# kabkabm/defensegan

Hardware: NVIDIA H100
Metric: reconstructed images/sec at R=10,L=200 (higher is better)
Workload: dtype f16

## Files before the change

### defensegan_b200/csrc/kernels_tc2.cuh

```cuda
#pragma once
#include "kernels_tc.cuh"
#include "tc_records.cuh"

namespace dgan {

constexpr int TC2_SMEM_MAX = 232448;
constexpr int TC2_TILE_BYTES = 128 * 128;
constexpr int TC2_BUF_COLS = 256;
constexpr int TC2_CONSUMERS = 256;
constexpr int TC2_THREADS = TC2_CONSUMERS + 128;
constexpr int TC2_PRODUCER_REGS = 40, TC2_CONSUMER_REGS = 232;
constexpr int TC2_STORE_ROWS = 16;

constexpr int TC2_MAX_PAIRS = 80;
struct Tc2Heads {
  uint32_t off[TC2_MAX_PAIRS + 1];
};

struct __align__(16) TcItem2 {
  uint16_t q[16];
  uint32_t n_acc;
};
static_assert(sizeof(TcItem2) == 48 && offsetof(TcItem2, n_acc) == 32, "the kernel's item loads");

__host__ __device__ constexpr int tc2_acc_stride(int n_tile) { return n_tile <= 32 ? 32 : (n_tile < 64 ? 64 : n_tile); }

__host__ __device__ constexpr bool tc2_tma_epilogue(int n_tile, int epi, int out_bytes) {
  return out_bytes == 2 && n_tile >= 64 && epi != EPI_FINAL_SIGMOID1 && epi != EPI_FINAL_TANH3 && epi != EPI_FINAL_SIGMOID1_W &&
         epi != EPI_FINAL_TANH3_W;
}

constexpr int TC2_REC_BATCH = 16;
constexpr int TC2_STAGING_BYTES = TC2_REC_BATCH * (int)sizeof(TcRec);
constexpr int TC2_MREC_BYTES = TC2_NSLOT * (int)sizeof(TcRec);

__host__ __device__ constexpr int tc2_epi_tiles(int n_tile, int epi, int out_bytes) {
  return tc2_tma_epilogue(n_tile, epi, out_bytes) ? 2 : 0;
}
__host__ __device__ constexpr int tc2_ksub(int K) { return K % 64 == 0 ? 4 : K / 16; }
__host__ __device__ constexpr int tc2_a_bytes(int ksub) { return 128 * 32 * ksub; }
__host__ __device__ constexpr int tc2_b_bytes(int n_tile, int ksub) { return n_tile * 32 * ksub; }
__host__ __device__ constexpr bool tc2_issues_zero_ops(int maxb, int ksub) { return maxb > 4 || (maxb > 1 && ksub < 4); }
__host__ __device__ constexpr int tc2_zero_bytes(int n_tile, int maxb, int ksub) { return maxb > 1 ? tc2_b_bytes(n_tile, ksub) : 0; }
__host__ __device__ constexpr int tc2_ring_bytes(int n_tile, int maxb, int ksub, int epi, int out_bytes) {
  const int epi_b = tc2_epi_tiles(n_tile, epi, out_bytes) * TC2_TILE_BYTES;
  const int raw = ((TC2_SMEM_MAX - 1024 - 256 - TC2_MREC_BYTES - TC2_STAGING_BYTES - epi_b - tc2_zero_bytes(n_tile, maxb, ksub)) / 1024) * 1024;
  return raw > TC2_RING_MAX_KB * 1024 ? TC2_RING_MAX_KB * 1024 : raw;
}

template <int N_TILE, int MAXB_, int KSUB_ = 4, int EPI = EPI_NONE, int OUT_BYTES = 2>
struct Tc2Cfg {
  static_assert(MAXB_ >= 1 && MAXB_ <= TC2_BUF_COLS / tc2_acc_stride(N_TILE), "more accumulator slots than columns");
  static_assert(KSUB_ >= 1 && KSUB_ <= 4, "k16 MMAs per op");
  static constexpr int KSUB = KSUB_;
  static constexpr int A_BYTES = tc2_a_bytes(KSUB);
  static constexpr int B_TILE = tc2_b_bytes(N_TILE, KSUB);
  static constexpr int A_SUB = 128 * 32, B_SUB = N_TILE * 32;
  static constexpr int MAXB = MAXB_;
  static constexpr int ACC_REGS = MAXB * N_TILE / 2;
  static constexpr bool TMA_EPI = tc2_tma_epilogue(N_TILE, EPI, OUT_BYTES);
  static constexpr int EPI_TILES = tc2_epi_tiles(N_TILE, EPI, OUT_BYTES);
  static constexpr int EPI_BYTES = EPI_TILES * TC2_TILE_BYTES;
  static constexpr int ZERO_BYTES = tc2_zero_bytes(N_TILE, MAXB, KSUB);
  static constexpr int RING_BYTES = tc2_ring_bytes(N_TILE, MAXB, KSUB, EPI, OUT_BYTES);
  static constexpr int SMEM_BYTES = RING_BYTES + ZERO_BYTES + EPI_BYTES + TC2_STAGING_BYTES + 1024 + 256 + TC2_MREC_BYTES;
};

#define TC2_KINDS(X)                                                                                                   \
  X(256, 1, 4, EPI_BIAS_RELU, __half) X(256, 1, 4, EPI_BIAS, __half) X(256, 1, 4, EPI_MASK, __half)                    \
  X(256, 1, 4, EPI_NONE, __half) X(256, 1, 4, EPI_NONE, float) X(256, 1, 4, EPI_BIAS, float)                           \
  X(128, 2, 4, EPI_BIAS_RELU, __half) X(128, 2, 4, EPI_BIAS, __half) X(128, 2, 4, EPI_MASK, __half)                    \
  X(128, 2, 4, EPI_NONE, __half) X(128, 2, 4, EPI_NONE, float) X(128, 2, 4, EPI_BIAS, float)                           \
  X(128, 1, 4, EPI_NONE, float)                                                                                        \
  X(64, 4, 4, EPI_BIAS_RELU, __half) X(64, 4, 4, EPI_BIAS, __half) X(64, 4, 4, EPI_MASK, __half)                      \
  X(64, 4, 4, EPI_NONE, __half) X(64, 4, 4, EPI_NONE, float) X(64, 4, 4, EPI_BIAS, float)                              \
  X(64, 4, 1, EPI_MASK, __half) X(64, 4, 1, EPI_NONE, __half) X(64, 4, 3, EPI_NONE, __half)                            \
  X(128, 2, 1, EPI_MASK, __half) X(128, 2, 1, EPI_NONE, __half) X(128, 2, 3, EPI_NONE, __half)                         \
  X(16, 8, 4, EPI_FINAL_SIGMOID1, __half) X(16, 4, 4, EPI_FINAL_SIGMOID1, __half) X(48, 4, 4, EPI_FINAL_TANH3, __half)   \
  X(16, 8, 4, EPI_NONE, float) X(48, 4, 4, EPI_NONE, float)                                                              \
  X(16, 8, 4, EPI_FINAL_SIGMOID1_W, __half) X(16, 4, 4, EPI_FINAL_SIGMOID1_W, __half) X(48, 4, 4, EPI_FINAL_TANH3_W, __half)

struct Tc2Kind { int n, maxb, ksub, epi, out_bytes; };
#define TC2_KIND_ROW(NT, MB, KS, EP, T) {NT, MB, KS, EP, (int)sizeof(T)},
static constexpr Tc2Kind kTc2Kinds[] = {TC2_KINDS(TC2_KIND_ROW)};
#undef TC2_KIND_ROW
constexpr bool tc2_kinds_fit_records() {
  for (const Tc2Kind& k : kTc2Kinds)
    if ((uint32_t)k.maxb > TcMmaRec::MaxB::mask || (uint32_t)k.ksub > TcMmaRec::Ksub::mask) return false;
  return true;
}
static_assert(tc2_kinds_fit_records(), "an instantiation's MAXB or KSUB does not fit the MMA record");
static inline bool tc2_has_kind(int n, int maxb, int ksub, int epi, int out_bytes) {
  for (const Tc2Kind& k : kTc2Kinds)
    if (k.n == n && k.maxb == maxb && k.ksub == ksub && k.epi == epi && k.out_bytes == out_bytes) return true;
  return false;
}

namespace ptx {
__device__ __forceinline__ void tma_store_3d(const CUtensorMap* map, uint32_t src, int c0, int c1, int c2) {
  asm volatile("cp.async.bulk.tensor.3d.global.shared::cta.tile.bulk_group [%0, {%2, %3, %4}], [%1];"
               ::"l"(map), "r"(src), "r"(c0), "r"(c1), "r"(c2) : "memory");
}
__device__ __forceinline__ void bulk_commit() { asm volatile("cp.async.bulk.commit_group;" ::: "memory"); }
__device__ __forceinline__ void bulk_wait_read1() { asm volatile("cp.async.bulk.wait_group.read 1;" ::: "memory"); }
__device__ __forceinline__ void bulk_wait_all0() { asm volatile("cp.async.bulk.wait_group 0;" ::: "memory"); }
__device__ __forceinline__ void fence_proxy_async_smem() { asm volatile("fence.proxy.async.shared::cta;" ::: "memory"); }
__device__ __forceinline__ uint32_t cluster_ctarank() {
  uint32_t r;
  asm volatile("mov.u32 %0, %%cluster_ctarank;" : "=r"(r));
  return r;
}
__device__ __forceinline__ void cluster_sync() {
  asm volatile("barrier.cluster.arrive.release.aligned;\n\tbarrier.cluster.wait.acquire.aligned;" ::: "memory");
}
__device__ __forceinline__ void tma_load_3d_mc2(uint32_t dst, const CUtensorMap* map, uint32_t bar, int c0, int c1, int c2) {
  asm volatile(
      "cp.async.bulk.tensor.3d.shared::cluster.global.mbarrier::complete_tx::bytes.multicast::cluster [%0], [%1, {%3, %4, %5}], [%2], %6;"
      ::"r"(dst), "l"(map), "r"(bar), "r"(c0), "r"(c1), "r"(c2), "h"((uint16_t)3) : "memory");
}
__device__ __forceinline__ void mbar_arrive_cluster(uint32_t local_bar, uint32_t cta) {
  asm volatile(
      "{\n\t.reg .b32 ra;\n\t"
      "mapa.shared::cluster.u32 ra, %0, %1;\n\t"
      "mbarrier.arrive.shared::cluster.b64 _, [ra];\n\t}" ::"r"(local_bar), "r"(cta) : "memory");
}
__device__ __forceinline__ void named_bar_sync(uint32_t id, uint32_t nthreads) {
  asm volatile("bar.sync %0, %1;" ::"r"(id), "r"(nthreads) : "memory");
}
__device__ __forceinline__ void st_shared_v4(uint32_t addr, uint32_t a, uint32_t b, uint32_t c, uint32_t d) {
  asm volatile("st.shared.v4.b32 [%0], {%1, %2, %3, %4};" ::"r"(addr), "r"(a), "r"(b), "r"(c), "r"(d) : "memory");
}
__device__ __forceinline__ void st_shared_u32(uint32_t addr, uint32_t v) { asm volatile("st.shared.b32 [%0], %1;" ::"r"(addr), "r"(v) : "memory"); }
__device__ __forceinline__ uint32_t ld_shared_u32(uint32_t addr) {
  uint32_t v;
  asm volatile("ld.shared.b32 %0, [%1];" : "=r"(v) : "r"(addr) : "memory");
  return v;
}
__device__ __forceinline__ uint2 ld_shared_v2(uint32_t addr) {
  uint2 v;
  asm volatile("ld.shared.v2.b32 {%0, %1}, [%2];" : "=r"(v.x), "=r"(v.y) : "r"(addr));
  return v;
}
__device__ __forceinline__ uint4 ld_shared_v4(uint32_t addr) {
  uint4 v;
  asm volatile("ld.shared.v4.b32 {%0, %1, %2, %3}, [%4];" : "=r"(v.x), "=r"(v.y), "=r"(v.z), "=r"(v.w) : "r"(addr));
  return v;
}
__device__ __forceinline__ uint4 ld_shared_v4_ordered(uint32_t addr) {
  uint4 v;
  asm volatile("ld.shared.v4.b32 {%0, %1, %2, %3}, [%4];" : "=r"(v.x), "=r"(v.y), "=r"(v.z), "=r"(v.w) : "r"(addr) : "memory");
  return v;
}
__device__ __forceinline__ void bulk_load(uint32_t dst, const void* src, uint32_t bytes, uint32_t bar) {
  asm volatile("cp.async.bulk.shared::cluster.global.mbarrier::complete_tx::bytes [%0], [%1], %2, [%3];"
               ::"r"(dst), "l"(src), "r"(bytes), "r"(bar) : "memory");
}
__device__ __forceinline__ void wgmma_wait1() { asm volatile("wgmma.wait_group.sync.aligned 1;" ::: "memory"); }
template <int R> __device__ __forceinline__ void setmaxnreg_inc() { asm volatile("setmaxnreg.inc.sync.aligned.u32 %0;" ::"n"(R)); }
template <int R> __device__ __forceinline__ void setmaxnreg_dec() { asm volatile("setmaxnreg.dec.sync.aligned.u32 %0;" ::"n"(R)); }
__device__ __forceinline__ bool elect_one() {
  uint32_t pred;
  asm volatile("{\n\t.reg .pred P1;\n\telect.sync _|P1, 0xffffffff;\n\tselp.u32 %0, 1, 0, P1;\n\t}" : "=r"(pred));
  return pred != 0;
}
}

__device__ __forceinline__ int tc2_item_at(const int* __restrict__ order, int k, int pair, int n_pairs, int n_slots) {
  return k < n_slots ? __ldg(order + (size_t)k * n_pairs + pair) : -1;
}

template <int NT, int MAXB, int KSUB, uint32_t MASK, int NREG>
__device__ __forceinline__ void tc2_mma_ops(float (&acc)[NREG], const uint32_t (&q)[6], uint64_t da0, uint64_t db0, uint32_t zoff) {
  constexpr uint32_t DA_K = KSUB == 4 ? 2u : (uint32_t)(128 * 32 >> 4), DB_K = KSUB == 4 ? 2u : (uint32_t)(NT * 32 >> 4);
#pragma unroll
  for (int a = 0; a < MAXB; ++a) {
    if (!((MASK >> a) & 1u)) continue;
    const uint32_t e = TcMmaRec::Ops::get(q[a / TcMmaRec::Ops::PER_WORD], a);
    const uint32_t bs = TcOp::Slot::get(e);
    const uint64_t da = da0 + (uint64_t)(TcOp::A::get(e) * (uint32_t)(tc2_a_bytes(KSUB) >> 4));
    const uint32_t boff = bs * (uint32_t)(tc2_b_bytes(NT, KSUB) >> 4);
    const uint64_t db = db0 + (uint64_t)(tc2_issues_zero_ops(MAXB, KSUB) && bs == (uint32_t)TC2_ZERO_SLOT ? zoff : boff);
    const uint32_t keep = TcOp::First::get(e) ^ 1u;
#pragma unroll
    for (int k = 0; k < KSUB; ++k) ptx::Wgmma<NT>::mma(acc + a * (NT / 2), da + DA_K * k, db + DB_K * k, k > 0 ? 1u : keep);
  }
  ptx::wgmma_commit();
}

template <int NT, int MAXB, int KSUB, int NREG>
__device__ __forceinline__ void tc2_mma_round(float (&acc)[NREG], const uint32_t (&q)[6], uint64_t da0, uint64_t db0, uint32_t zoff) {
  if constexpr (tc2_issues_zero_ops(MAXB, KSUB) || MAXB == 1) {
    tc2_mma_ops<NT, MAXB, KSUB, (1u << MAXB) - 1u>(acc, q, da0, db0, zoff);
  } else {
    static_assert(MAXB <= TcMmaRec::Ops::PER_WORD, "a round's op bytes share the queue's first word");
    uint32_t set = 0;
#pragma unroll
    for (int a = 0; a < MAXB; ++a)
      set |= (TcOp::Slot::get(TcMmaRec::Ops::get(q[0], a)) != (uint32_t)TC2_ZERO_SLOT ? 1u : 0u) << a;
    switch (set) {
#define TC2_ROUND_VARIANT(M) \
  case M:                    \
    if constexpr (M < (1u << MAXB)) tc2_mma_ops<NT, MAXB, KSUB, M>(acc, q, da0, db0, zoff); \
    break;
      TC2_ROUND_VARIANT(1u) TC2_ROUND_VARIANT(2u) TC2_ROUND_VARIANT(3u) TC2_ROUND_VARIANT(4u) TC2_ROUND_VARIANT(5u)
      TC2_ROUND_VARIANT(6u) TC2_ROUND_VARIANT(7u) TC2_ROUND_VARIANT(8u) TC2_ROUND_VARIANT(9u) TC2_ROUND_VARIANT(10u)
      TC2_ROUND_VARIANT(11u) TC2_ROUND_VARIANT(12u) TC2_ROUND_VARIANT(13u) TC2_ROUND_VARIANT(14u) TC2_ROUND_VARIANT(15u)
#undef TC2_ROUND_VARIANT
      default: __builtin_unreachable();
    }
  }
}

template <int MAXB>
__device__ __forceinline__ void tc2_pop_round(uint32_t (&q)[6]) {
  using Ops = TcMmaRec::Ops;
  static_assert(Ops::WORDS == 6, "the op queue holds every op word");
  if constexpr (MAXB >= Ops::PER_WORD) {
#pragma unroll
    for (int i = 0; i < 6; ++i) q[i] = (i + MAXB / Ops::PER_WORD < 6) ? q[i + MAXB / Ops::PER_WORD] : 0u;
  } else {
#pragma unroll
    for (int i = 0; i < 5; ++i) q[i] = __funnelshift_r(q[i], q[i + 1], Ops::BITS * MAXB);
    q[5] >>= Ops::BITS * MAXB;
  }
}

#ifdef DGAN_PROBE
constexpr int TC2_PROBE_WORDS = 16;
__device__ unsigned long long g_tc2_probe[48][160][TC2_PROBE_WORDS];
__device__ __forceinline__ unsigned long long probe_gtime() {
  unsigned long long t;
  asm volatile("mov.u64 %0, %%globaltimer;" : "=l"(t));
  return t;
}
__device__ __forceinline__ long long probe_clock_after(uint32_t w0) {
  long long t;
  asm volatile("{\n\t.reg .pred p;\n\tsetp.ge.s32 p, %1, 0;\n\tmov.u64 %0, 0;\n\t@p mov.u64 %0, %%clock64;\n\t}" : "=l"(t) : "r"(w0) : "memory");
  return t;
}
__host__ __device__ constexpr int tc2_probe_key(int n_tile, int epi, int out_bytes) {
  return (n_tile == 256 ? 0 : n_tile == 128 ? 1 : n_tile == 64 ? 2 : n_tile == 48 ? 3 : 4) * 8 + (out_bytes == 4 ? 6 : (epi < 4 ? epi : epi - 4));
}
#endif

template <int N_TILE, int MAXB, int KSUB, int EPI, typename TOUT>
__global__ void __cluster_dims__(2, 1, 1) __launch_bounds__(TC2_THREADS, 1)
tc_bsgemm2_kernel(const __grid_constant__ CUtensorMap tm_a, const __grid_constant__ CUtensorMap tm_b,
                  const __grid_constant__ CUtensorMap tm_out,
                  const TcItem2* __restrict__ items, const TcRec* __restrict__ stream_p,
                  const TcRec* __restrict__ stream_m, const __grid_constant__ Tc2Heads heads,
                  const int* __restrict__ eitems, int n_slots,
                  TOUT* __restrict__ out, int n_pad, const float* __restrict__ bias, int bias_pstride, const TcFinalArgs fa) {
  using Cfg = Tc2Cfg<N_TILE, MAXB, KSUB, EPI, (int)sizeof(TOUT)>;
  constexpr bool TMA_EPI = Cfg::TMA_EPI;
  constexpr bool WEIGHTED = (EPI == EPI_FINAL_SIGMOID1_W || EPI == EPI_FINAL_TANH3_W);
  constexpr bool FINAL = (EPI == EPI_FINAL_SIGMOID1 || EPI == EPI_FINAL_TANH3 || WEIGHTED);
  constexpr bool SIGMOID1 = (EPI == EPI_FINAL_SIGMOID1 || EPI == EPI_FINAL_SIGMOID1_W);
  constexpr bool HAS_BIAS = (EPI == EPI_BIAS_RELU || EPI == EPI_BIAS);
  constexpr int B_TILE = Cfg::B_TILE, A_BYTES = Cfg::A_BYTES;
  constexpr int PRODUCER = TC2_CONSUMERS / 32;
  extern __shared__ uint8_t smem_raw[];
#ifdef DGAN_PROBE
  const long long probe_t_start = clock64();
  const unsigned long long probe_g_start = probe_gtime();
  long long probe_wait_full = 0, probe_issue = 0, probe_wait1 = 0, probe_wait0 = 0, probe_epi = 0;
  unsigned probe_rec = 0, probe_head = 0, probe_steps = 0;
#endif
  const uint32_t smem_base = (ptx::smem_u32(smem_raw) + 1023u) & ~1023u;
  const uint32_t zero_base = smem_base + Cfg::RING_BYTES;
  const uint32_t epi_base = zero_base + Cfg::ZERO_BYTES;
  const uint32_t stg_base = epi_base + Cfg::EPI_BYTES;
  const uint32_t bar_base = stg_base + TC2_STAGING_BYTES;
  const uint32_t bar_full = bar_base, bar_empty = bar_base + 64, mrec_base = bar_base + 256;

  const int warp = threadIdx.x >> 5, lane = threadIdx.x & 31;
  const uint32_t rank = ptx::cluster_ctarank();
  const int pair = blockIdx.x >> 1, n_pairs = gridDim.x >> 1;
  const uint32_t rbeg = heads.off[pair], rend = heads.off[pair + 1];

  uint4 mine = make_uint4(0, 0, 0, 0);
  if (warp == PRODUCER) {
    if (2 * rbeg + lane < 2 * rend) mine = __ldg(reinterpret_cast<const uint4*>(stream_p + rbeg) + lane);
    if (lane == 0) {
      ptx::prefetch_tmap(&tm_a);
      ptx::prefetch_tmap(&tm_b);
      if (TMA_EPI) ptx::prefetch_tmap(&tm_out);
      for (int s = 0; s < TC2_NSLOT; ++s) {
        ptx::mbar_init(bar_full + 8 * s, 1);
        ptx::mbar_init(bar_empty + 8 * s, 2 * TC2_CONSUMERS / 32);
      }
      ptx::fence_barrier_init();
    }
  }
  if constexpr (Cfg::ZERO_BYTES > 0 && tc2_issues_zero_ops(MAXB, KSUB)) {
    if (threadIdx.x < TC2_CONSUMERS) {
      for (uint32_t i = threadIdx.x; i < (uint32_t)Cfg::ZERO_BYTES / 16u; i += TC2_CONSUMERS) ptx::st_shared_v4(zero_base + 16u * i, 0u, 0u, 0u, 0u);
      ptx::fence_proxy_async_smem();
    }
  }
  ptx::cluster_sync();
#ifdef DGAN_PROBE
  const long long probe_t_entry = clock64();
#endif
  pdl_launch_dependents();
  pdl_wait();
#ifdef DGAN_PROBE
  const long long probe_t_go = clock64();
  unsigned probe_h0 = (unsigned)probe_t_go;
  bool probe_new_item = true;
#endif

  if (warp >= PRODUCER) {
    ptx::setmaxnreg_dec<TC2_PRODUCER_REGS>();
    if (warp == PRODUCER) {
      const TcRec* __restrict__ stream = stream_p;
      uint32_t it = 0;
      const uint32_t ring = stg_base;
      for (uint32_t base = rbeg; base < rend; base += TC2_REC_BATCH) {
        ptx::st_shared_v4(ring + lane * 16u, mine.x, mine.y, mine.z, mine.w);
        __syncwarp();
        if (2 * (base + TC2_REC_BATCH) + lane < 2 * rend) mine = __ldg(reinterpret_cast<const uint4*>(stream + base + TC2_REC_BATCH) + lane);
        const uint32_t cnt = min((uint32_t)TC2_REC_BATCH, rend - base);
        for (uint32_t i = 0; i < cnt; ++i, ++it) {
          const uint4 r0 = ptx::ld_shared_v4(ring + i * 32u);
          const uint2 r1 = ptx::ld_shared_v2(ring + i * 32u + 16u);
          const uint32_t slot = it & (TC2_NSLOT - 1);
          using P = TcProducerRec;
          const int kc = P::Kc::get(r0.x), nA = P::NA::get(r0.x), nB = P::NB::get(r0.x);
          const uint32_t dep = (r0.x >> P::Dep::shift) & P::Dep::mask;
          const int row0 = (2 * (int)P::Mp::get(r0.y) + (int)rank) * kRowTile;
          if (it >= dep) ptx::mbar_wait(bar_empty + 8 * ((it - dep) & (TC2_NSLOT - 1)), ((it - dep) >> 3) & 1);
          if (dep != TC2_NSLOT && it >= TC2_NSLOT) ptx::mbar_wait(bar_empty + 8 * slot, ((it - TC2_NSLOT) >> 3) & 1);
          const uint32_t full = bar_full + 8 * slot;
          const uint32_t sa = smem_base + (P::Off::get(r0.x) << 10);
          if (ptx::elect_one()) {
            ptx::mbar_expect_tx(full, (uint32_t)(nA * A_BYTES + nB * B_TILE) + (uint32_t)sizeof(TcRec));
            ptx::bulk_load(mrec_base + slot * (uint32_t)sizeof(TcRec), stream_m + rbeg + it, (uint32_t)sizeof(TcRec), full);
#pragma unroll
            for (int a = 0; a < TC2_MAX_A; ++a) {
              if (a >= nA) break;
              const int p = (int)P::Pix::get(a < P::Pix::PER_WORD ? r0.z : r0.w, a);
              if constexpr (KSUB == 4) {
                ptx::tma_load_3d(sa + a * A_BYTES, &tm_a, full, kc * 64, row0, p);
              } else {
#pragma unroll
                for (int k = 0; k < KSUB; ++k)
                  ptx::tma_load_3d(sa + a * A_BYTES + k * Cfg::A_SUB, &tm_a, full, (kc * KSUB + k) * 16, row0, p);
              }
            }
            const uint32_t sb = sa + nA * A_BYTES;
#pragma unroll
            for (int b = 0; b < TC2_MAX_BSLOTS; ++b) {
              if (b >= nB) break;
              const uint32_t t = P::Tile::get(b < P::Tile::PER_WORD ? r1.x : r1.y, b);
              if constexpr (KSUB == 4) {
                ptx::tma_load_3d_mc2(sb + b * B_TILE + rank * (B_TILE / 2), &tm_b, full, kc * 64, (int)rank * (N_TILE / 2), (int)t);
              } else {
#pragma unroll
                for (int k = 0; k < KSUB; ++k)
                  ptx::tma_load_3d_mc2(sb + b * B_TILE + k * Cfg::B_SUB + rank * (Cfg::B_SUB / 2), &tm_b, full, (kc * KSUB + k) * 16,
                                       (int)rank * (N_TILE / 2), (int)t);
              }
            }
          }
          __syncwarp();
        }
        __syncwarp();
      }
      for (uint32_t j = it > TC2_NSLOT ? it - TC2_NSLOT : 0; j < it; ++j) ptx::mbar_wait(bar_empty + 8 * (j & (TC2_NSLOT - 1)), (j >> 3) & 1);
    }
  } else {
    ptx::setmaxnreg_inc<TC2_CONSUMER_REGS>();
    const int wg = warp >> 2, wl = warp & 3;
    const int r_lo = wg * 64 + wl * 16 + (lane >> 2);
    float acc[Cfg::ACC_REGS];
#pragma unroll
    for (int i = 0; i < Cfg::ACC_REGS; ++i) acc[i] = 0.f;
    uint32_t item_count = 0, store_count = 0;
    uint32_t ri = rbeg, it = 0;
    while (ri < rend) {
      const int item_e = tc2_item_at(eitems, (int)item_count, pair, n_pairs, n_slots);
      const TcItem2* ip = items + tc2_item_window(item_e);
      const int n_acc = (int)__ldg(&ip->n_acc);
      const uint32_t q_mine = lane < 16 ? (uint32_t)__ldg(&ip->q[lane]) : 0u;
      uint32_t flags;
      do {
        const uint32_t slot = it & (TC2_NSLOT - 1), phase = (it >> 3) & 1;
#ifdef DGAN_PROBE
        const long long probe_w0 = clock64();
        if (probe_new_item) probe_head += (unsigned)probe_w0 - probe_h0;
        probe_new_item = false;
#endif
        ptx::mbar_wait(bar_full + 8 * slot, phase);
#ifdef DGAN_PROBE
        const long long probe_w1 = clock64();
        probe_wait_full += probe_w1 - probe_w0;
        if (it == 0 && threadIdx.x == 0) g_tc2_probe[tc2_probe_key(N_TILE, EPI, (int)sizeof(TOUT))][blockIdx.x][7] = probe_gtime();
#endif
        const uint4 r0 = ptx::ld_shared_v4_ordered(mrec_base + slot * (uint32_t)sizeof(TcRec));
        const uint4 r1 = ptx::ld_shared_v4_ordered(mrec_base + slot * (uint32_t)sizeof(TcRec) + 16u);
        flags = TcMmaRec::Flags::get(r0.x);
#ifdef DGAN_PROBE
        const unsigned probe_rec_step = (unsigned)probe_clock_after(r0.x) - (unsigned)probe_w1;
        probe_rec += probe_rec_step;
#endif
        const int nA = TcMmaRec::NA::get(r0.x), n_rounds = TcMmaRec::Rounds::get(r0.x);
        const uint32_t sa = smem_base + (TcMmaRec::Off::get(r0.x) << 10);
        const uint64_t da0 = KSUB == 4 ? make_smem_desc_sw128(sa + (uint32_t)wg * 64u * 128u) : make_smem_desc_sw32(sa + (uint32_t)wg * 64u * 32u);
        const uint32_t sb = sa + (uint32_t)nA * A_BYTES;
        const uint64_t db0 = KSUB == 4 ? make_smem_desc_sw128(sb) : make_smem_desc_sw32(sb);
        const uint32_t zoff = (zero_base - sb) >> 4;
        uint32_t q[6] = {r0.z, r0.w, r1.x, r1.y, r1.z, r1.w};
#ifdef DGAN_PROBE
        long long probe_step_wait = 0;
#endif
        ptx::fence_operands(acc);
        ptx::wgmma_fence();
        for (int r = 0; r < n_rounds; ++r) {
          tc2_mma_round<N_TILE, Cfg::MAXB, KSUB>(acc, q, da0, db0, zoff);
          tc2_pop_round<Cfg::MAXB>(q);
#ifdef DGAN_PROBE
          const long long probe_c0 = clock64();
#endif
          ptx::wgmma_wait1();
#ifdef DGAN_PROBE
          probe_step_wait += clock64() - probe_c0;
#endif
          if (r == 0) {
            __syncwarp();
            if (!(flags & TcMmaRec::FIRST) && lane < 2) ptx::mbar_arrive_cluster(bar_empty + 8 * ((it - 1) & (TC2_NSLOT - 1)), (uint32_t)lane);
          }
        }
        ptx::fence_operands(acc);
#ifdef DGAN_PROBE
        probe_wait1 += probe_step_wait;
        probe_issue += clock64() - probe_w1 - probe_step_wait - probe_rec_step;
#endif
        ++ri; ++it;
      } while (!(flags & TcMmaRec::LAST));
#ifdef DGAN_PROBE
      const long long probe_d0 = clock64();
#endif
      ptx::wgmma_wait0();
      ptx::fence_operands(acc);
#ifdef DGAN_PROBE
      const long long probe_e0 = clock64();
      probe_wait0 += probe_e0 - probe_d0;
#endif
      __syncwarp();
      if (lane < 2) ptx::mbar_arrive_cluster(bar_empty + 8 * ((it - 1) & (TC2_NSLOT - 1)), (uint32_t)lane);

      const int mp = tc2_item_mp(item_e);
      auto q_of = [&](int a) { return (int)__shfl_sync(0xffffffffu, q_mine, a); };
      const int tile_row0 = (2 * mp + (int)rank) * kRowTile;
      const size_t n_lo = (size_t)(tile_row0 + r_lo);
      if constexpr (FINAL) {
        constexpr int CO = SIGMOID1 ? 1 : 3;
        const int hwc = fa.w_out * fa.w_out * CO;
        float bsv[CO];
#pragma unroll
        for (int co = 0; co < CO; ++co) bsv[co] = __ldg(bias + co);
#pragma unroll
        for (int a = 0; a < Cfg::MAXB; ++a) {
          if (a >= n_acc) break;
          const int blk = q_of(a);
          const int by = blk / fa.nbx, bx = blk % fa.nbx;
#pragma unroll
          for (int h = 0; h < 2; ++h) {
            const size_t n = n_lo + 8 * h;
            const int img = min((int)(n / fa.R), fa.B - 1);
            float lsum = 0.f;
#pragma unroll
            for (int j = 0; j < N_TILE / 8; ++j) {
              const int col = j * 8 + (lane & 3) * 2;
              const int li = col / (4 * CO), e = col % (4 * CO);
              const size_t off = (size_t)((4 * by + li) * fa.w_out + 4 * bx) * CO + e;
              float2 xv = make_float2(0.f, 0.f);
              if (fa.x != nullptr) xv = __ldg(reinterpret_cast<const float2*>(fa.x + (size_t)img * hwc + off));
              float2 wv = make_float2(1.f, 1.f);
              if (WEIGHTED) wv = __ldg(reinterpret_cast<const float2*>(fa.xw + (size_t)img * hwc + off));
              float yv[2], dv[2];
#pragma unroll
              for (int c = 0; c < 2; ++c) {
                const float pre = acc[a * (N_TILE / 2) + j * 4 + h * 2 + c] + bsv[(e + c) % CO];
                float yy, dact;
                if (SIGMOID1) { yy = __fdividef(1.f, 1.f + __expf(-pre)); dact = yy * (1.f - yy); }
                else { const float t = __expf(-2.f * fabsf(pre)); yy = copysignf(__fdividef(1.f - t, 1.f + t), pre); dact = 1.f - yy * yy; }
                yv[c] = yy;
                float d = 0.f;
                if (WEIGHTED) {
                  d = yy - (c ? xv.y : xv.x);
                  const float ew = (c ? wv.y : wv.x) * d;
                  lsum = fmaf(ew, d, lsum);
                  d = ew;
                } else if (fa.x != nullptr) { d = yy - (c ? xv.y : xv.x); lsum = fmaf(d, d, lsum); }
                dv[c] = d * dact * fa.gscale;
              }
              if (fa.write_y) *reinterpret_cast<float2*>(fa.y + n * hwc + off) = make_float2(yv[0], yv[1]);
              if (fa.x != nullptr)
                *reinterpret_cast<uint32_t*>(reinterpret_cast<__half*>(out) + ((size_t)blk * n_pad + n) * N_TILE + col) = pack_half2(dv[0], dv[1]);
            }
            lsum += __shfl_xor_sync(0xffffffffu, lsum, 1);
            lsum += __shfl_xor_sync(0xffffffffu, lsum, 2);
            if (fa.x != nullptr && fa.write_y && (lane & 3) == 0) fa.loss_part[(size_t)blk * n_pad + n] = lsum;
          }
        }
      } else if constexpr (TMA_EPI) {
        constexpr int G = N_TILE / 64;
        const int GT = fa.out_ld >> 6;
        const int row_w = tile_row0 + wg * 64 + wl * 16;
        const uint32_t s_warp = epi_base + (uint32_t)warp * 4096u;
        const uint32_t swz = (uint32_t)(lane >> 2);
#pragma unroll
        for (int a = 0; a < Cfg::MAXB; ++a) {
          if (a >= n_acc) break;
          const int q = q_of(a);
#pragma unroll
          for (int g = 0; g < G; ++g) {
            unsigned long long mk[2] = {~0ull, ~0ull}, bits[2] = {0ull, 0ull};
            if (EPI == EPI_MASK) {
#pragma unroll
              for (int h = 0; h < 2; ++h) mk[h] = __ldg(fa.mb_in + ((size_t)q * n_pad + n_lo + 8 * h) * GT + g);
            }
            uint32_t pk[2][8];
#pragma unroll
            for (int j = 0; j < 8; ++j) {
              const int cl = j * 8 + (lane & 3) * 2;
              float2 bv = make_float2(0.f, 0.f);
              if (HAS_BIAS) bv = __ldg(reinterpret_cast<const float2*>(bias + (size_t)q * bias_pstride + g * 64 + cl));
#pragma unroll
              for (int h = 0; h < 2; ++h) {
                float v0 = acc[a * (N_TILE / 2) + (g * 8 + j) * 4 + h * 2];
                float v1 = acc[a * (N_TILE / 2) + (g * 8 + j) * 4 + h * 2 + 1];
                if (HAS_BIAS) { v0 += bv.x; v1 += bv.y; }
                if (EPI == EPI_BIAS_RELU) {
                  v0 = fmaxf(v0, 0.f); v1 = fmaxf(v1, 0.f);
                  bits[h] |= ((unsigned long long)(v0 > 0.f) << cl) | ((unsigned long long)(v1 > 0.f) << (cl + 1));
                }
                if (EPI == EPI_MASK) {
                  if (!((mk[h] >> cl) & 1ull)) v0 = 0.f;
                  if (!((mk[h] >> (cl + 1)) & 1ull)) v1 = 0.f;
                }
                pk[h][j] = pack_half2(v0, v1);
              }
            }
            const uint32_t buf = s_warp + (store_count & 1u) * 2048u;
            if (lane == 0) ptx::bulk_wait_read1();
            __syncwarp();
#pragma unroll
            for (int h = 0; h < 2; ++h)
#pragma unroll
              for (int j = 0; j < 8; ++j)
                ptx::st_shared_u32(buf + (swz + 8u * h) * 128u + (((uint32_t)j ^ swz) << 4) + (uint32_t)(lane & 3) * 4u, pk[h][j]);
            ptx::fence_proxy_async_smem();
            __syncwarp();
            if (lane == 0) {
              ptx::tma_store_3d(&tm_out, buf, fa.col0 + g * 64, row_w, q);
              ptx::bulk_commit();
            }
            ++store_count;
            if (EPI == EPI_BIAS_RELU && fa.mb_out != nullptr) {
#pragma unroll
              for (int h = 0; h < 2; ++h) {
                bits[h] |= __shfl_xor_sync(0xffffffffu, bits[h], 1);
                bits[h] |= __shfl_xor_sync(0xffffffffu, bits[h], 2);
              }
              if ((lane & 3) < 2) fa.mb_out[((size_t)q * n_pad + n_lo + 8 * (lane & 1)) * GT + g] = (lane & 1) ? bits[1] : bits[0];
            }
          }
        }
      } else {
#pragma unroll
        for (int a = 0; a < Cfg::MAXB; ++a) {
          if (a >= n_acc) break;
          const int q = q_of(a);
#pragma unroll
          for (int j = 0; j < N_TILE / 8; ++j) {
            const int col = j * 8 + (lane & 3) * 2;
            float2 bv = make_float2(0.f, 0.f);
            if (HAS_BIAS) bv = __ldg(reinterpret_cast<const float2*>(bias + (size_t)q * bias_pstride + col));
#pragma unroll
            for (int h = 0; h < 2; ++h) {
              float v0 = acc[a * (N_TILE / 2) + j * 4 + h * 2] + bv.x, v1 = acc[a * (N_TILE / 2) + j * 4 + h * 2 + 1] + bv.y;
              if (EPI == EPI_BIAS_RELU) { v0 = fmaxf(v0, 0.f); v1 = fmaxf(v1, 0.f); }
              const size_t o = ((size_t)q * n_pad + n_lo + 8 * h) * fa.out_ld + col;
              if (sizeof(TOUT) == 4) *reinterpret_cast<float2*>(reinterpret_cast<float*>(out) + o) = make_float2(v0, v1);
              else *reinterpret_cast<uint32_t*>(reinterpret_cast<__half*>(out) + o) = pack_half2(v0, v1);
            }
          }
        }
      }
      if (EPI == EPI_NONE && sizeof(TOUT) == 4 && fa.m_counter != nullptr) {
        const uint32_t flag_addr = bar_base + 200;
        const unsigned rt = 2u * (unsigned)mp + rank;
        __threadfence();
        ptx::named_bar_sync(3, TC2_CONSUMERS);
        if (threadIdx.x == 0) {
          const unsigned ticket = atomicAdd(fa.m_counter + rt, 1u);
          ptx::st_shared_u32(flag_addr, ticket == (unsigned)TC_LINEAR_SPLIT - 1u ? 1u : 0u);
        }
        ptx::named_bar_sync(3, TC2_CONSUMERS);
        if (ptx::ld_shared_u32(flag_addr) != 0u) {
          __threadfence();
          const float* __restrict__ gp = reinterpret_cast<const float*>(out);
          const size_t base = (size_t)rt * kRowTile * N_TILE;
          const int tid = threadIdx.x;
          constexpr int STRIDE = 4 * TC2_CONSUMERS, UNR = 4;
          for (int e0 = tid * 4; e0 < kRowTile * N_TILE; e0 += UNR * STRIDE) {
            float4 gs[UNR], vv[UNR], zz[UNR];
#pragma unroll
            for (int u = 0; u < UNR; ++u) {
              const size_t i = base + (size_t)(e0 + u * STRIDE);
              gs[u] = __ldcg(reinterpret_cast<const float4*>(gp + i));
              vv[u] = *reinterpret_cast<const float4*>(fa.mv + i);
              zz[u] = *reinterpret_cast<const float4*>(fa.mz + i);
            }
            float4 t[TC_LINEAR_SPLIT - 1][UNR];
#pragma unroll
            for (int pp = 1; pp < TC_LINEAR_SPLIT; ++pp)
#pragma unroll
              for (int u = 0; u < UNR; ++u)
                t[pp - 1][u] = __ldcg(reinterpret_cast<const float4*>(gp + base + (size_t)(e0 + u * STRIDE) + (size_t)pp * fa.m_count));
#pragma unroll
            for (int pp = 1; pp < TC_LINEAR_SPLIT; ++pp)
#pragma unroll
              for (int u = 0; u < UNR; ++u) { gs[u].x += t[pp - 1][u].x; gs[u].y += t[pp - 1][u].y; gs[u].z += t[pp - 1][u].z; gs[u].w += t[pp - 1][u].w; }
#pragma unroll
            for (int u = 0; u < UNR; ++u) {
              const size_t i = base + (size_t)(e0 + u * STRIDE);
              float4 v4 = vv[u], z4 = zz[u];
              v4.x = fmaf(fa.m_mu, v4.x, fa.m_gmul * gs[u].x); v4.y = fmaf(fa.m_mu, v4.y, fa.m_gmul * gs[u].y);
              v4.z = fmaf(fa.m_mu, v4.z, fa.m_gmul * gs[u].z); v4.w = fmaf(fa.m_mu, v4.w, fa.m_gmul * gs[u].w);
              z4.x -= fa.m_lr * v4.x; z4.y -= fa.m_lr * v4.y; z4.z -= fa.m_lr * v4.z; z4.w -= fa.m_lr * v4.w;
              *reinterpret_cast<float4*>(fa.mv + i) = v4;
              *reinterpret_cast<float4*>(fa.mz + i) = z4;
              if (fa.mz_h != nullptr)
                *reinterpret_cast<uint2*>(fa.mz_h + i) = make_uint2(pack_half2(z4.x, z4.y), pack_half2(z4.z, z4.w));
            }
          }
          if (tid == 0) fa.m_counter[rt] = 0u;
        }
      }
#ifdef DGAN_PROBE
      const long long probe_e1 = clock64();
      probe_epi += probe_e1 - probe_e0;
      probe_h0 = (unsigned)probe_e1;
      probe_new_item = true;
      probe_steps = it;
#endif
      ++item_count;
    }
    if (TMA_EPI && lane == 0) ptx::bulk_wait_all0();
  }

#ifdef DGAN_PROBE
  {
    constexpr int key = tc2_probe_key(N_TILE, EPI, (int)sizeof(TOUT));
    if (threadIdx.x == 0) {
      atomicAdd(&g_tc2_probe[key][blockIdx.x][3], (unsigned long long)probe_wait_full);
      atomicAdd(&g_tc2_probe[key][blockIdx.x][8], (unsigned long long)probe_issue);
      atomicAdd(&g_tc2_probe[key][blockIdx.x][9], (unsigned long long)probe_wait1);
      atomicAdd(&g_tc2_probe[key][blockIdx.x][10], (unsigned long long)probe_wait0);
      atomicAdd(&g_tc2_probe[key][blockIdx.x][11], (unsigned long long)probe_epi);
    }
    __syncthreads();
    if (threadIdx.x == 0) {
      atomicAdd(&g_tc2_probe[key][blockIdx.x][12], (unsigned long long)probe_rec);
      atomicAdd(&g_tc2_probe[key][blockIdx.x][13], (unsigned long long)probe_head);
      atomicAdd(&g_tc2_probe[key][blockIdx.x][15], (unsigned long long)probe_steps);
      if (probe_steps != 0) atomicAdd(&g_tc2_probe[key][blockIdx.x][14], (unsigned long long)((unsigned)clock64() - probe_h0));
      atomicAdd(&g_tc2_probe[key][blockIdx.x][0], (unsigned long long)(clock64() - probe_t_go));
      atomicAdd(&g_tc2_probe[key][blockIdx.x][1], 1ull);
      atomicAdd(&g_tc2_probe[key][blockIdx.x][2], (unsigned long long)(probe_t_go - probe_t_entry));
      atomicAdd(&g_tc2_probe[key][blockIdx.x][4], (unsigned long long)(probe_t_entry - probe_t_start));
      g_tc2_probe[key][blockIdx.x][5] = probe_g_start;
      g_tc2_probe[key][blockIdx.x][6] = probe_gtime();
    }
  }
#endif
  ptx::cluster_sync();
}

struct Tc2Schedule {
  TcItem2* items = nullptr;
  TcRec* stream_p = nullptr;
  TcRec* stream_m = nullptr;
  Tc2Heads heads{};
  int* eitems = nullptr;
  int n_slots = 0, n_pairs = 0;
  int maxb = 1;
};
static uint32_t tc2_box_k(int K) { return tc2_ksub(K) == 4 ? 64u : 16u; }
struct TcDir {
  std::string name, kind;
  int N = 0, K = 0, P_in = 0, P_out = 0, n_tiles = 0;
  PairTable tab;
  int h_grid = 0, w_grid = 0;
  int max_acc = 1;
  int epi = EPI_NONE, out_bytes = 2, bias_pstride = 0;
  int ld = 0, col0 = 0, out_ld = 0;
  int n_real = 0;
  std::string base_kind;
  __half* w = nullptr;
  CUtensorMap tm_b{};
  int force_maxb = 0;
  std::vector<std::pair<int, Tc2Schedule>> by_mpairs;
};

static int tc2_maxb(int N) { return TC2_BUF_COLS / tc2_acc_stride(N); }

struct Tc2HostStep {
  int kc = 0, nA = 0, nB = 0, n_rounds = 0;
  int a_pix[TC2_MAX_A] = {0, 0, 0, 0};
  uint8_t b_ent[TC2_MAX_BSLOTS] = {0};
  uint8_t ops[TC2_OP_BYTES] = {0};
  int n_real = 0;
  int bytes = 0;
};
struct Tc2HostItem {
  TcItem2 hdr{};
  std::vector<Tc2HostStep> steps;
  double stage_bytes = 0.0;
  long long n_ops = 0;
  long long n_issued = 0;
};

static void tc2_build_item(const PairTable& tab, const std::vector<int>& qs, int N, int K, int max_b, int max_a,
                           int step_max_bytes, Tc2HostItem* out) {
  const int ksub = tc2_ksub(K), kch = K / (16 * ksub), a_bytes = tc2_a_bytes(ksub), b_tile = tc2_b_bytes(N, ksub);
  out->hdr = TcItem2{};
  out->hdr.n_acc = (uint32_t)qs.size();
  for (size_t a = 0; a < qs.size(); ++a) out->hdr.q[a] = (uint16_t)qs[a];
  out->steps.clear();
  std::vector<std::pair<int, std::vector<std::pair<int, int>>>> by_p;
  for (size_t a = 0; a < qs.size(); ++a)
    for (int e = tab.off[qs[a]]; e < tab.off[qs[a] + 1]; ++e) {
      const int p = tab.pairs[e].x, t = tab.pairs[e].y;
      size_t g = 0;
      for (; g < by_p.size(); ++g)
        if (by_p[g].first == p) break;
      if (g == by_p.size()) by_p.push_back({p, {}});
      by_p[g].second.push_back({t, (int)a});
    }
  std::sort(by_p.begin(), by_p.end(), [](const auto& l, const auto& r) { return l.first < r.first; });
  for (auto& g : by_p)
    std::stable_sort(g.second.begin(), g.second.end(), [](const auto& l, const auto& r) { return l.second < r.second; });
  std::vector<std::pair<int, std::vector<std::pair<int, int>>>> px;
  const int ent_cap = std::min(TC2_MAX_BSLOTS, std::max(1, (step_max_bytes - a_bytes) / b_tile));
  for (auto& g : by_p)
    for (size_t b0 = 0; b0 < g.second.size(); b0 += (size_t)ent_cap)
      px.push_back({g.first, std::vector<std::pair<int, int>>(g.second.begin() + b0,
                                                               g.second.begin() + std::min(g.second.size(), b0 + (size_t)ent_cap))});
  const int max_rounds = TC2_OP_BYTES / max_b;
  struct Group { size_t i0, i1; };
  std::vector<Group> groups;
  {
    size_t i0 = 0;
    while (i0 < px.size()) {
      size_t i1 = i0;
      std::vector<int> staged;
      int cnt[8] = {0, 0, 0, 0, 0, 0, 0, 0};
      auto have = [&](int t) { return std::find(staged.begin(), staged.end(), t) != staged.end(); };
      while (i1 < px.size() && (int)(i1 - i0) < max_a) {
        int fresh = 0;
        std::vector<int> fresh_tiles;
        int c2[8];
        std::copy(cnt, cnt + 8, c2);
        int rounds = 0;
        for (auto& ta : px[i1].second) {
          if (!have(ta.first) && std::find(fresh_tiles.begin(), fresh_tiles.end(), ta.first) == fresh_tiles.end()) {
            fresh_tiles.push_back(ta.first); ++fresh;
          }
          ++c2[ta.second];
        }
        for (int a = 0; a < 8; ++a) rounds = std::max(rounds, c2[a]);
        const int nA = (int)(i1 - i0) + 1, nB = (int)staged.size() + fresh;
        const bool dup_pixel = (i1 > i0 && px[i1].first == px[i1 - 1].first);
        if (i1 > i0 && (dup_pixel || nB > TC2_MAX_BSLOTS || rounds > max_rounds ||
                        nA * a_bytes + nB * b_tile > step_max_bytes))
          break;
        for (int t : fresh_tiles) staged.push_back(t);
        std::copy(c2, c2 + 8, cnt);
        ++i1;
      }
      groups.push_back({i0, i1});
      i0 = i1;
    }
  }
  uint32_t seen = 0;
  for (size_t gi = 0; gi < groups.size(); ++gi) {
    const Group& G = groups[gi];
    Tc2HostStep st;
    st.nA = (int)(G.i1 - G.i0);
    std::fill(st.ops, st.ops + TC2_OP_BYTES, TC2_PAD_OP);
    int slot_of[32], cnt[8] = {0, 0, 0, 0, 0, 0, 0, 0};
    for (int t = 0; t < 32; ++t) slot_of[t] = -1;
    for (size_t i = G.i0; i < G.i1; ++i) {
      st.a_pix[i - G.i0] = px[i].first;
      for (auto& ta : px[i].second) {
        const int t = ta.first, acc = ta.second;
        if (slot_of[t] < 0) {
          slot_of[t] = st.nB;
          st.b_ent[st.nB++] = (uint8_t)t;
        }
        const bool first = !(seen & (1u << acc));
        const int r = cnt[acc]++;
        st.ops[r * max_b + acc] = TcOp{(uint32_t)(i - G.i0), (uint32_t)slot_of[t], first ? 1u : 0u}.encode();
        st.n_rounds = std::max(st.n_rounds, r + 1);
        st.n_real += 1;
        seen |= 1u << acc;
      }
    }
    st.bytes = st.nA * a_bytes + st.nB * b_tile;
    out->steps.push_back(st);
  }
  const size_t n_groups = out->steps.size();
  for (int kc = 1; kc < kch; ++kc)
    for (size_t gi = 0; gi < n_groups; ++gi) {
      Tc2HostStep sk = out->steps[gi];
      sk.kc = kc;
      for (int o = 0; o < TC2_OP_BYTES; ++o) sk.ops[o] = (uint8_t)TcOp::First::put(sk.ops[o], 0u);
      out->steps.push_back(sk);
    }
  out->stage_bytes = 0.0;
  out->n_ops = 0;
  out->n_issued = 0;
  for (auto& stp : out->steps) {
    out->stage_bytes += stp.bytes;
    out->n_ops += (long long)stp.n_rounds * max_b;
    out->n_issued += tc2_issues_zero_ops(max_b, ksub) ? (long long)stp.n_rounds * max_b : (long long)stp.n_real;
  }
}

static void tc2_enumerate_windows(int h_grid, int w_grid, int wh, int ww, int sy, int sx, std::vector<std::vector<int>>* wins) {
  wins->clear();
  for (int by = 0; by < h_grid; by += wh * sy)
    for (int bx = 0; bx < w_grid; bx += ww * sx)
      for (int ry = 0; ry < sy; ++ry)
        for (int rx = 0; rx < sx; ++rx) {
          std::vector<int> qs;
          for (int i = 0; i < wh; ++i)
            for (int j = 0; j < ww; ++j) {
              const int y = by + ry + i * sy, x = bx + rx + j * sx;
              if (y < h_grid && x < w_grid) qs.push_back(y * w_grid + x);
            }
          if (!qs.empty()) wins->push_back(qs);
        }
}

#ifndef DGAN_STEP_MAX_KB
#define DGAN_STEP_MAX_KB 48
#endif
#ifndef DGAN_STEP_MAX_KB_N64
#define DGAN_STEP_MAX_KB_N64 64
#endif
#ifndef DGAN_COST_EPI_KB
#define DGAN_COST_EPI_KB 24.0
#endif
#ifndef DGAN_COST_FIXED_KB
#define DGAN_COST_FIXED_KB 48.0
#endif
#ifndef DGAN_COST_NS_PER_KB
#define DGAN_COST_NS_PER_KB 6.8
#endif
#ifndef DGAN_COST_OP_NS
#define DGAN_COST_OP_NS 103.0
#endif
#ifndef DGAN_COST_STEP_NS
#define DGAN_COST_STEP_NS 942.0
#endif
#ifndef DGAN_COST_OP_MIN_N
#define DGAN_COST_OP_MIN_N 32
#endif
#ifndef TC2_REFINE_BUDGET
#define TC2_REFINE_BUDGET (1LL << 26)
#endif

struct Tc2Plan {
  int shape[4] = {1, 1, 1, 1};
  int n_slots = 0, n_pairs = 0;
  std::vector<TcItem2> hdrs;
  std::vector<TcRec> stream_p, stream_m;
  std::vector<uint32_t> stream_off;
  std::vector<int> eitems;
  long long n_mma = 0, n_pad = 0, n_issued = 0, n_steps = 0, n_bytes = 0;
  double load_max = 0.0, load_mean = 0.0;
  double op_ns_max = 0.0;
  double op_ns_issued_max = 0.0;
  int maxb = 1, ring_bytes = 0;
  int ksub = 4;
};

static double tc2_op_ns(int N, int ksub) {
  return DGAN_COST_OP_NS * (double)std::max(N, DGAN_COST_OP_MIN_N) / 64.0 * (double)ksub / 4.0;
}

static int tc2_search(int N, int K, const PairTable& tab, int h_grid, int w_grid, int max_acc, int force_maxb, int epi,
                      int out_bytes, int n_mpairs, int n_pairs, const int* force_shape, Tc2Plan* plan,
                      std::vector<Tc2HostItem>* best_items, std::vector<std::vector<int>>* best_lists) {
  const int max_a = TC2_MAX_A;
  const int step_kb = (N == 64 && K == 128) ? DGAN_STEP_MAX_KB_N64 : DGAN_STEP_MAX_KB;
  const int ksub = tc2_ksub(K);
  const double op_ns = tc2_op_ns(N, ksub);
  double best_cost = 1e300;
  plan->maxb = 0;
  std::vector<std::vector<int>> wins;
  for (const Tc2Kind& kind : kTc2Kinds) {
    if (kind.n != N || kind.ksub != ksub || kind.epi != epi || kind.out_bytes != out_bytes) continue;
    if (force_maxb > 0 && kind.maxb != force_maxb) continue;
    const int mb = kind.maxb, ring = tc2_ring_bytes(N, mb, ksub, epi, out_bytes);
    const int step_max = std::min((ring / 3) & ~1023, step_kb * 1024);
    for (int wh = 1; wh <= 2; ++wh)
      for (int ww = 1; ww <= 8; ++ww)
        for (int sy = 1; sy <= (wh > 1 ? 2 : 1); ++sy)
          for (int sx = 1; sx <= (ww > 1 ? 2 : 1); ++sx) {
            if (wh * ww > std::min(max_acc, mb) || wh > h_grid || ww > std::max(w_grid, 1)) continue;
            if (force_shape != nullptr && (wh != force_shape[0] || ww != force_shape[1] || sy != force_shape[2] || sx != force_shape[3])) continue;
            tc2_enumerate_windows(h_grid, std::max(w_grid, 1), wh, ww, sy, sx, &wins);
            std::vector<Tc2HostItem> items(wins.size());
            for (size_t i = 0; i < wins.size(); ++i) tc2_build_item(tab, wins[i], N, K, mb, max_a, step_max, &items[i]);
            std::vector<double> icost(items.size());
            auto cost_item = [&](const Tc2HostItem& it) {
              return DGAN_COST_NS_PER_KB / 1024.0 *
                         (it.stage_bytes + DGAN_COST_EPI_KB * 1024.0 * it.hdr.n_acc * std::max(1, N / 64) + DGAN_COST_FIXED_KB * 1024.0) +
                     op_ns * (double)it.n_ops + DGAN_COST_STEP_NS * (double)it.steps.size();
            };
            std::stable_sort(items.begin(), items.end(), [](const Tc2HostItem& l, const Tc2HostItem& r) { return l.stage_bytes > r.stage_bytes; });
            for (size_t i = 0; i < items.size(); ++i) icost[i] = cost_item(items[i]);
            const long long total = (long long)items.size() * n_mpairs;
            std::vector<double> load((size_t)n_pairs, 0.0);
            std::vector<std::vector<int>> lists((size_t)n_pairs);
            for (long long idx = 0; idx < total; ++idx) {
              size_t best = 0;
              for (size_t pr = 1; pr < (size_t)n_pairs; ++pr)
                if (load[pr] < load[best]) best = pr;
              load[best] += icost[(size_t)(idx / n_mpairs)];
              lists[best].push_back((int)idx);
            }
            auto cost_of = [&](int idx) { return icost[(size_t)(idx / n_mpairs)]; };
            long long work = 0;
            for (int iter = 0; iter < 4096 && work < TC2_REFINE_BUDGET; ++iter) {
              const size_t P = (size_t)(std::max_element(load.begin(), load.end()) - load.begin());
              double best_peak = load[P];
              size_t bq = P; int bi = -1, bj = -1;
              for (size_t Q = 0; Q < (size_t)n_pairs; ++Q) {
                if (Q == P) continue;
                work += (long long)lists[P].size() * (long long)(1 + lists[Q].size());
                for (size_t i = 0; i < lists[P].size(); ++i) {
                  const double ci = cost_of(lists[P][i]);
                  double peak = std::max(load[P] - ci, load[Q] + ci);
                  if (peak < best_peak - 1e-9) { best_peak = peak; bq = Q; bi = (int)i; bj = -1; }
                  for (size_t j = 0; j < lists[Q].size(); ++j) {
                    const double cj = cost_of(lists[Q][j]);
                    if (cj >= ci) continue;
                    peak = std::max(load[P] - ci + cj, load[Q] + ci - cj);
                    if (peak < best_peak - 1e-9) { best_peak = peak; bq = Q; bi = (int)i; bj = (int)j; }
                  }
                }
              }
              if (bi < 0) break;
              const int it_i = lists[P][(size_t)bi];
              const double ci = cost_of(it_i);
              if (bj < 0) {
                lists[P].erase(lists[P].begin() + bi);
                lists[bq].push_back(it_i);
                load[P] -= ci; load[bq] += ci;
// ... 285 lines not shown
```

Before: 2714.

## Prefetch epilogue inputs and next item descriptor before the MMA loop

Consumer warps now load the next work item's descriptor one item ahead, and issue the epilogue's global loads (mask bits, per-pixel bias, final-stage x/xw pairs) before waiting on the MMA pipeline. Channel bias is staged once into shared memory, and mask and bias values are redistributed with warp shuffles instead of per-lane global loads. The aim is to hide global-load latency in the epilogue behind the wgmma mainloop. The cost is extra registers held across the mainloop in a kernel already running at high register counts, which risks spills. Probe counters for input and staging time are also added.

New measurement: 2804 (median of 6 runs). +3.3%, better.

```diff
diff --git a/defensegan_b200/csrc/kernels_tc2.cuh b/defensegan_b200/csrc/kernels_tc2.cuh
--- a/defensegan_b200/csrc/kernels_tc2.cuh
+++ b/defensegan_b200/csrc/kernels_tc2.cuh
@@ -226,7 +226,7 @@
 }
 
 #ifdef DGAN_PROBE
-constexpr int TC2_PROBE_WORDS = 16;
+constexpr int TC2_PROBE_WORDS = 18;
 __device__ unsigned long long g_tc2_probe[48][160][TC2_PROBE_WORDS];
 __device__ __forceinline__ unsigned long long probe_gtime() {
   unsigned long long t;
@@ -237,6 +237,15 @@
   long long t;
   asm volatile("{\n\t.reg .pred p;\n\tsetp.ge.s32 p, %1, 0;\n\tmov.u64 %0, 0;\n\t@p mov.u64 %0, %%clock64;\n\t}" : "=l"(t) : "r"(w0) : "memory");
   return t;
+}
+__device__ __forceinline__ long long probe_clock_after64(unsigned long long v) {
+  long long t;
+  asm volatile("{\n\t.reg .pred p;\n\tsetp.eq.u64 p, %1, 0;\n\t@p mov.u64 %0, %%clock64;\n\t@!p mov.u64 %0, %%clock64;\n\t}"
+               : "=l"(t) : "l"(v) : "memory");
+  return t;
+}
+__device__ __forceinline__ unsigned long long probe_bits(float2 v) {
+  return ((unsigned long long)__float_as_uint(v.y) << 32) | __float_as_uint(v.x);
 }
 __host__ __device__ constexpr int tc2_probe_key(int n_tile, int epi, int out_bytes) {
   return (n_tile == 256 ? 0 : n_tile == 128 ? 1 : n_tile == 64 ? 2 : n_tile == 48 ? 3 : 4) * 8 + (out_bytes == 4 ? 6 : (epi < 4 ? epi : epi - 4));
@@ -263,7 +272,7 @@
 #ifdef DGAN_PROBE
   const long long probe_t_start = clock64();
   const unsigned long long probe_g_start = probe_gtime();
-  long long probe_wait_full = 0, probe_issue = 0, probe_wait1 = 0, probe_wait0 = 0, probe_epi = 0;
+  long long probe_wait_full = 0, probe_issue = 0, probe_wait1 = 0, probe_wait0 = 0, probe_epi = 0, probe_in = 0, probe_stage = 0;
   unsigned probe_rec = 0, probe_head = 0, probe_steps = 0;
 #endif
   const uint32_t smem_base = (ptx::smem_u32(smem_raw) + 1023u) & ~1023u;
@@ -378,11 +387,89 @@
     for (int i = 0; i < Cfg::ACC_REGS; ++i) acc[i] = 0.f;
     uint32_t item_count = 0, store_count = 0;
     uint32_t ri = rbeg, it = 0;
+    auto item_desc = [&](int e, int& n, uint32_t& qm) {
+      n = 0; qm = 0u;
+      if (e < 0) return;
+      const TcItem2* ip = items + tc2_item_window(e);
+      n = (int)__ldg(&ip->n_acc);
+      if (lane < 16) qm = (uint32_t)__ldg(&ip->q[lane]);
+    };
+    int e_cur = tc2_item_at(eitems, 0, pair, n_pairs, n_slots), e_nx = tc2_item_at(eitems, 1, pair, n_pairs, n_slots), n_acc_cur;
+    uint32_t q_cur;
+    item_desc(e_cur, n_acc_cur, q_cur);
+    constexpr bool BIAS_CH = HAS_BIAS && TMA_EPI && N_TILE < 256, BIAS_PX = HAS_BIAS && TMA_EPI && !BIAS_CH;
+    static_assert(!BIAS_CH || (Cfg::ZERO_BYTES >= N_TILE * 4 && !tc2_issues_zero_ops(MAXB, KSUB)), "the bias copy's space");
+    static_assert(!BIAS_PX || MAXB == 1, "a per-pixel bias is held for one accumulator");
+    if constexpr (BIAS_CH) {
+      if (threadIdx.x < N_TILE / 2) {
+        const float2 b2 = __ldg(reinterpret_cast<const float2*>(bias) + threadIdx.x);
+        ptx::st_shared_u32(zero_base + 8u * threadIdx.x, __float_as_uint(b2.x));
+        ptx::st_shared_u32(zero_base + 8u * threadIdx.x + 4u, __float_as_uint(b2.y));
+      }
+      ptx::named_bar_sync(4, TC2_CONSUMERS);
+    }
+    constexpr int CO = SIGMOID1 ? 1 : 3, FJ = FINAL ? N_TILE / 8 : 1;
+    constexpr bool FINAL_PREFETCH = !(WEIGHTED && N_TILE > 32);
+    constexpr int FINAL_HELD = FINAL && N_TILE <= 32 && !(WEIGHTED && MAXB > 4) ? MAXB : 1;
+    const int hwc = fa.w_out * fa.w_out * CO;
+    float bsv[CO];
+    if constexpr (FINAL) {
+#pragma unroll
+      for (int co = 0; co < CO; ++co) bsv[co] = __ldg(bias + co);
+    }
     while (ri < rend) {
-      const int item_e = tc2_item_at(eitems, (int)item_count, pair, n_pairs, n_slots);
-      const TcItem2* ip = items + tc2_item_window(item_e);
-      const int n_acc = (int)__ldg(&ip->n_acc);
-      const uint32_t q_mine = lane < 16 ? (uint32_t)__ldg(&ip->q[lane]) : 0u;
+      const int item_e = e_cur, n_acc = n_acc_cur;
+      const uint32_t q_mine = q_cur;
+      const int mp = tc2_item_mp(item_e);
+      const int tile_row0 = (2 * mp + (int)rank) * kRowTile;
+      const size_t n_lo = (size_t)(tile_row0 + r_lo);
+      constexpr int G_UNITS = TMA_EPI ? N_TILE / 64 : 1;
+      static_assert(EPI != EPI_MASK || MAXB * G_UNITS == 4, "one mask unit per lane of a quad");
+      unsigned long long mk_pre[2] = {~0ull, ~0ull};
+      if constexpr (EPI == EPI_MASK) {
+        const int ua = (lane & 3) / G_UNITS, ug = (lane & 3) % G_UNITS;
+        const size_t qa = (size_t)__shfl_sync(0xffffffffu, q_mine, ua);
+        if (ua < n_acc) {
+#pragma unroll
+          for (int h = 0; h < 2; ++h) mk_pre[h] = __ldg(fa.mb_in + (qa * n_pad + n_lo + 8 * h) * (size_t)(fa.out_ld >> 6) + ug);
+        }
+      }
+      float2 bias_px[BIAS_PX ? G_UNITS : 1];
+      if constexpr (BIAS_PX) {
+        const size_t q0 = (size_t)__shfl_sync(0xffffffffu, q_mine, 0);
+        if (n_acc > 0) {
+#pragma unroll
+          for (int g = 0; g < G_UNITS; ++g)
+            bias_px[g] = __ldg(reinterpret_cast<const float2*>(bias + q0 * bias_pstride + (g * 8 + (lane >> 2)) * 8 + (lane & 3) * 2));
+        }
+      }
+      auto final_pairs = [&](int a, int h, float2 (&xv)[FJ], float2 (&wv)[FJ]) {
+        const int blk = (int)__shfl_sync(0xffffffffu, q_mine, a);
+        const int by = blk / fa.nbx, bx = blk % fa.nbx;
+        const int img = min((int)((n_lo + 8 * h) / fa.R), fa.B - 1);
+#pragma unroll
+        for (int j = 0; j < FJ; ++j) {
+          const int col = j * 8 + (lane & 3) * 2;
+          const int li = col / (4 * CO), e = col % (4 * CO);
+          const size_t off = (size_t)((4 * by + li) * fa.w_out + 4 * bx) * CO + e;
+          xv[j] = make_float2(0.f, 0.f);
+          if (fa.x != nullptr) xv[j] = __ldg(reinterpret_cast<const float2*>(fa.x + (size_t)img * hwc + off));
+          wv[j] = make_float2(1.f, 1.f);
+          if (WEIGHTED) wv[j] = __ldg(reinterpret_cast<const float2*>(fa.xw + (size_t)img * hwc + off));
+        }
+      };
+      float2 xp[FINAL_HELD][2][FJ], wp[FINAL_HELD][2][FJ];
+      if constexpr (FINAL && FINAL_PREFETCH) {
+#pragma unroll
+        for (int a = 0; a < FINAL_HELD; ++a) {
+          if (a >= n_acc) break;
+          final_pairs(a, 0, xp[a][0], wp[a][0]);
+          final_pairs(a, 1, xp[a][1], wp[a][1]);
+        }
+      }
+      item_desc(e_nx, n_acc_cur, q_cur);
+      e_cur = e_nx;
+      e_nx = tc2_item_at(eitems, (int)item_count + 2, pair, n_pairs, n_slots);
       uint32_t flags;
       do {
         const uint32_t slot = it & (TC2_NSLOT - 1), phase = (it >> 3) & 1;
@@ -450,35 +537,37 @@
       __syncwarp();
       if (lane < 2) ptx::mbar_arrive_cluster(bar_empty + 8 * ((it - 1) & (TC2_NSLOT - 1)), (uint32_t)lane);
 
-      const int mp = tc2_item_mp(item_e);
       auto q_of = [&](int a) { return (int)__shfl_sync(0xffffffffu, q_mine, a); };
-      const int tile_row0 = (2 * mp + (int)rank) * kRowTile;
-      const size_t n_lo = (size_t)(tile_row0 + r_lo);
       if constexpr (FINAL) {
-        constexpr int CO = SIGMOID1 ? 1 : 3;
-        const int hwc = fa.w_out * fa.w_out * CO;
-        float bsv[CO];
-#pragma unroll
-        for (int co = 0; co < CO; ++co) bsv[co] = __ldg(bias + co);
 #pragma unroll
         for (int a = 0; a < Cfg::MAXB; ++a) {
           if (a >= n_acc) break;
           const int blk = q_of(a);
           const int by = blk / fa.nbx, bx = blk % fa.nbx;
+#ifdef DGAN_PROBE
+          const long long probe_a0 = clock64();
+#endif
 #pragma unroll
           for (int h = 0; h < 2; ++h) {
+            float2 xa[FJ], wa[FJ];
+            if constexpr (FINAL_PREFETCH) {
+#pragma unroll
+              for (int j = 0; j < FJ; ++j) { xa[j] = xp[a % FINAL_HELD][h][j]; wa[j] = wp[a % FINAL_HELD][h][j]; }
+              if (FINAL_HELD == 1 && a + 1 < Cfg::MAXB && a + 1 < n_acc) final_pairs(a + 1, h, xp[0][h], wp[0][h]);
+            } else {
+              final_pairs(a, h, xa, wa);
+            }
+#ifdef DGAN_PROBE
+            if (h == 0) probe_in += probe_clock_after64(probe_bits(xa[0]) ^ probe_bits(wa[0])) - probe_a0;
+#endif
             const size_t n = n_lo + 8 * h;
-            const int img = min((int)(n / fa.R), fa.B - 1);
             float lsum = 0.f;
 #pragma unroll
             for (int j = 0; j < N_TILE / 8; ++j) {
               const int col = j * 8 + (lane & 3) * 2;
               const int li = col / (4 * CO), e = col % (4 * CO);
               const size_t off = (size_t)((4 * by + li) * fa.w_out + 4 * bx) * CO + e;
-              float2 xv = make_float2(0.f, 0.f);
-              if (fa.x != nullptr) xv = __ldg(reinterpret_cast<const float2*>(fa.x + (size_t)img * hwc + off));
-              float2 wv = make_float2(1.f, 1.f);
-              if (WEIGHTED) wv = __ldg(reinterpret_cast<const float2*>(fa.xw + (size_t)img * hwc + off));
+              const float2 xv = xa[j], wv = wa[j];
               float yv[2], dv[2];
 #pragma unroll
               for (int c = 0; c < 2; ++c) {
@@ -517,17 +606,33 @@
           const int q = q_of(a);
 #pragma unroll
           for (int g = 0; g < G; ++g) {
+#ifdef DGAN_PROBE
+            const long long probe_u0 = clock64();
+#endif
             unsigned long long mk[2] = {~0ull, ~0ull}, bits[2] = {0ull, 0ull};
             if (EPI == EPI_MASK) {
 #pragma unroll
-              for (int h = 0; h < 2; ++h) mk[h] = __ldg(fa.mb_in + ((size_t)q * n_pad + n_lo + 8 * h) * GT + g);
+              for (int h = 0; h < 2; ++h) mk[h] = __shfl_sync(0xffffffffu, mk_pre[h], (lane & ~3) | (a * G + g));
+#ifdef DGAN_PROBE
+              probe_in += probe_clock_after64(mk[0] ^ mk[1]) - probe_u0;
+#endif
             }
             uint32_t pk[2][8];
 #pragma unroll
             for (int j = 0; j < 8; ++j) {
               const int cl = j * 8 + (lane & 3) * 2;
               float2 bv = make_float2(0.f, 0.f);
-              if (HAS_BIAS) bv = __ldg(reinterpret_cast<const float2*>(bias + (size_t)q * bias_pstride + g * 64 + cl));
+              if constexpr (BIAS_CH) {
+                const uint2 b2 = ptx::ld_shared_v2(zero_base + (uint32_t)(g * 64 + cl) * 4u);
+                bv = make_float2(__uint_as_float(b2.x), __uint_as_float(b2.y));
+              }
+              if constexpr (BIAS_PX) {
+                bv.x = __shfl_sync(0xffffffffu, bias_px[g].x, j * 4 + (lane & 3));
+                bv.y = __shfl_sync(0xffffffffu, bias_px[g].y, j * 4 + (lane & 3));
+              }
+#ifdef DGAN_PROBE
+              if (HAS_BIAS && j == 0) probe_in += probe_clock_after64(probe_bits(bv)) - probe_u0;
+#endif
 #pragma unroll
               for (int h = 0; h < 2; ++h) {
                 float v0 = acc[a * (N_TILE / 2) + (g * 8 + j) * 4 + h * 2];
@@ -545,8 +650,14 @@
               }
             }
             const uint32_t buf = s_warp + (store_count & 1u) * 2048u;
+#ifdef DGAN_PROBE
+            const long long probe_s0 = clock64();
+#endif
             if (lane == 0) ptx::bulk_wait_read1();
             __syncwarp();
+#ifdef DGAN_PROBE
+            probe_stage += clock64() - probe_s0;
+#endif
 #pragma unroll
             for (int h = 0; h < 2; ++h)
 #pragma unroll
@@ -662,6 +773,8 @@
       atomicAdd(&g_tc2_probe[key][blockIdx.x][9], (unsigned long long)probe_wait1);
       atomicAdd(&g_tc2_probe[key][blockIdx.x][10], (unsigned long long)probe_wait0);
       atomicAdd(&g_tc2_probe[key][blockIdx.x][11], (unsigned long long)probe_epi);
+      atomicAdd(&g_tc2_probe[key][blockIdx.x][16], (unsigned long long)probe_in);
+      atomicAdd(&g_tc2_probe[key][blockIdx.x][17], (unsigned long long)probe_stage);
     }
     __syncthreads();
     if (threadIdx.x == 0) {
```
